# musyoku/chainer-speech-recognition

Hardware: AMD Instinct MI355X
Metric: utterances/sec (T=1000, 40x3 feat, |V|~3000) CTC train step (higher is better)
Workload: dtype bf16

## Files before the change

### chainer-speech-recognition_amd/asr/_lib.py

```python
import ctypes
import os

import torch

_HERE = os.path.dirname(os.path.abspath(__file__))
_ACT = os.environ.get("ASR_ACT", "").lower()
LIB_PATH = os.environ.get("ASR_HIP_LIB") or os.path.join(os.path.dirname(_HERE),
                                                        "libasr_hip_f16.so" if _ACT in ("f16", "fp16", "float16", "half") else "libasr_hip.so")

_lib = None


def act_dtype():
    return torch.float16 if lib().asr_act_dtype() else torch.bfloat16


def debug_flag(key, default):
    for item in os.environ.get("ASR_DEBUG", "").split(","):
        k, _, v = item.strip().partition("=")
        if k == key and v:
            return int(v)
    return default

c_void_p, c_int, c_float, c_size_t = ctypes.c_void_p, ctypes.c_int, ctypes.c_float, ctypes.c_size_t
# ... 39 lines not shown
    "asr_conv_nt_8pn_ok": (c_int, [c_void_p, c_void_p, c_int, c_void_p, c_int, c_void_p] + [c_int] * 9),
    "asr_conv_nt_8pn": (c_int, [c_void_p, c_void_p, c_void_p, c_int, c_void_p, c_int, c_void_p] + [c_int] * 12),
    "asr_conv_direct_ok": (c_int, [c_int] * 11),
    "asr_conv_direct_nt": (c_int, [c_void_p, c_void_p, c_void_p, c_int, c_void_p, c_void_p] + [c_int] * 12),
    "asr_conv_mp_ok": (c_int, [c_int] * 5),
    "asr_conv_mp_fwd": (c_int, [c_void_p] * 3 + [c_int] + [c_void_p] * 3 + [c_int] * 11),
    "asr_conv_mp_bwd_workspace": (c_longlong, [c_int] * 5),
    "asr_conv_mp_bwd": (c_int, [c_void_p] * 7 + [c_int] * 12),
    "asr_pack_input_pad": (c_int, [c_void_p, c_void_p, c_int] + [c_longlong] * 4 + [c_int] * 5 + [c_void_p]),
    "asr_conv_weight_pack_bwd": (c_int, [c_void_p] * 3 + [c_int] * 4),
    "asr_gemm_tn_acc": (c_int, [c_void_p, c_void_p, c_int, c_void_p, c_int, c_void_p, c_int] + [c_int] * 3),
    "asr_gemm_tn_acc_group": (c_int, [c_void_p, c_int] + [c_void_p] * 9),
    "asr_gemm_tn_8ph_ok": (c_int, [c_void_p, c_int, c_void_p, c_int, c_void_p, c_int, c_int, c_int, c_int]),
    "asr_gemm_tn_acc_group_8ph": (c_int, [c_void_p, c_int] + [c_void_p] * 9),
    "asr_cast_bf16": (c_int, [c_void_p, c_void_p, c_void_p, c_int, c_int, c_int]),
    "asr_cast_bf16_many": (c_int, [c_void_p, c_void_p, c_int, c_longlong]),
    "asr_bf16_to_f32": (c_int, [c_void_p, c_void_p, c_void_p, c_longlong]),
    "asr_permute4": (c_int, [c_void_p, c_void_p, c_int, c_void_p, c_int] + [c_int] * 4 + [c_longlong] * 4),
    "asr_im2col": (c_int, [c_void_p, c_void_p, c_int] + [c_longlong] * 4 + [c_int] * 10 + [c_void_p]),
    "asr_col2im": (c_int, [c_void_p, c_void_p] + [c_int] * 10 + [c_void_p]),
    "asr_activation_fwd": (c_int, [c_void_p] * 3 + [c_longlong, c_int, c_float]),
    "asr_activation_bwd": (c_int, [c_void_p] * 4 + [c_longlong, c_int, c_float]),
    "asr_glu_fwd": (c_int, [c_void_p] * 3 + [c_longlong, c_int]),
    "asr_glu_bwd": (c_int, [c_void_p] * 4 + [c_longlong, c_int]),
    "asr_dropout": (c_int, [c_void_p] * 3 + [c_longlong, c_float, ctypes.c_uint]),
    "asr_conv_weight_pack": (c_int, [c_void_p] * 3 + [c_int] * 6),
    "asr_conv_weight_grad_unpack": (c_int, [c_void_p] * 3 + [c_int] * 6),
    "asr_conv_tn_acc": (c_int, [c_void_p, c_void_p, c_int, c_void_p, c_void_p] + [c_int] * 12),
    "asr_conv_tn_8ph_ok": (c_int, [c_void_p, c_int, c_void_p, c_void_p] + [c_int] * 10),
    "asr_conv_tn_acc_8ph": (c_int, [c_void_p, c_void_p, c_int, c_void_p, c_void_p] + [c_int] * 12),
    "asr_conv_tn_copies": (c_int, [c_int] * 4),
    "asr_conv_tn_acc_copies": (c_int, [c_void_p, c_void_p, c_int, c_void_p, c_void_p] + [c_int] * 13),
    "asr_conv_weight_grad_unpack_copies": (c_int, [c_void_p, c_void_p, c_int, c_void_p] + [c_int] * 6),
    "asr_maxout2_fwd": (c_int, [c_void_p] * 3 + [c_longlong]),
    "asr_maxout2_bwd": (c_int, [c_void_p] * 4 + [c_longlong]),
    "asr_maxout2_pool_fwd": (c_int, [c_void_p] * 3 + [c_longlong, c_int, c_int, c_int]),
    "asr_maxout2_pool_bwd": (c_int, [c_void_p] * 4 + [c_longlong, c_int, c_int, c_int]),
    "asr_maxout2_pool_bwd_db": (c_int, [c_void_p] * 5 + [c_longlong, c_int, c_int, c_int]),
    "asr_maxout2_pool_bwd_db_ok": (c_int, [c_int]),
    "asr_maxpool_h_fwd": (c_int, [c_void_p] * 3 + [c_longlong, c_int, c_int, c_int]),
    "asr_maxpool_h_bwd": (c_int, [c_void_p] * 4 + [c_longlong, c_int, c_int, c_int]),
    "asr_add_bf16": (c_int, [c_void_p] * 4 + [c_longlong]),
    "asr_colsum_acc": (c_int, [c_void_p, c_void_p, c_int, c_longlong, c_int, c_int, c_void_p]),
    "asr_layernorm_fwd": (c_int, [c_void_p, c_void_p, c_int, c_void_p, c_int] + [c_void_p] * 4 + [c_longlong, c_int, c_int]),
    "asr_layernorm_fwd_lse": (c_int, [c_void_p] * 8 + [c_longlong, c_int]),
    "asr_layernorm_fwd_lse_ok": (c_int, [c_int, c_int]),
    "asr_layernorm_bwd": (c_int, [c_void_p, c_void_p, c_int, c_void_p, c_int] + [c_void_p] * 3 + [c_void_p, c_int, c_void_p, c_void_p,
                                  c_longlong, c_int, c_int]),
    "asr_layernorm_bwd_rows_ws_bytes": (c_longlong, [c_longlong, c_int]),
    "asr_layernorm_bwd_rows": (c_int, [c_void_p] * 7 + [c_int, c_void_p, c_void_p, c_longlong, c_int, c_int, c_void_p, c_longlong]),
    "asr_layernorm_fold_partials": (c_int, [c_void_p, c_void_p, c_int, c_int, c_int, c_void_p, c_void_p, c_void_p]),
    "asr_layernorm_ctc_bwd_ws_bytes": (c_longlong, [c_int, c_int, c_int]),
    "asr_layernorm_ctc_bwd": (c_int, [c_void_p] * 7 + [c_int, c_void_p, c_void_p, c_int, c_int, c_int, c_void_p, c_longlong, c_int] +
                              [c_void_p, c_int, c_int, c_void_p, c_void_p, c_int, c_float] * 2 + [c_void_p]),
    "asr_weightnorm_fwd": (c_int, [c_void_p] * 5 + [c_int, c_int]),
    "asr_weightnorm_bwd": (c_int, [c_void_p] * 7 + [c_int, c_int]),
    "asr_channel_stats": (c_int, [c_void_p, c_void_p, c_longlong, c_int, c_void_p, c_void_p]),
    "asr_channel_affine": (c_int, [c_void_p] * 5 + [c_longlong, c_int]),
    "asr_weightnorm_init": (c_int, [c_void_p] * 5 + [c_int]),
    "asr_gru_sync_bytes": (c_size_t, [c_int] * 3),
    "asr_gru_fwd_accepts_bf16_gi": (c_int, [c_int] * 5),
    "asr_gru_gates_f16_ok": (c_int, [c_int] * 5),
    "asr_gru_fwd": (c_int, [c_void_p, c_void_p, c_int] + [c_void_p] * 6 + [c_int] * 4 + [c_void_p, c_int, c_void_p, c_int]),
    "asr_gru_bwd": (c_int, [c_void_p] * 10 + [c_int] * 4 + [c_void_p, c_int, c_void_p, c_void_p, c_int]),
    "asr_gru_fwd_state": (c_int, [c_void_p] * 9 + [c_int] * 4 + [c_void_p]),
    "asr_gru_bwd_state": (c_int, [c_void_p] * 13 + [c_int] * 4 + [c_void_p, c_void_p]),
# ... 71 lines not shown
```

### chainer-speech-recognition_amd/asr/_ops.py

```python
import os

import torch

from . import _lib
from ._lib import check, ptr, stream

BF16 = _lib.act_dtype()
F32 = torch.float32


def _is_bf16(t):
    if t.dtype == BF16:
        return 1
    if t.dtype == F32:
        return 0
    raise TypeError("expected float32 or bfloat16, got %s" % t.dtype)


def gemm_nt(a, b, bias=None, out_dtype=BF16, out=None):
    assert a.dtype == BF16 and b.dtype == BF16 and a.dim() == 2 and b.dim() == 2
    assert a.stride(1) == 1 and b.stride(1) == 1 and a.shape[1] == b.shape[1]
    M, K = a.shape
    N = b.shape[0]
    if out is None:
# ... 112 lines not shown
    return dx


def conv_weight_pack(W, transpose=False, Kp=None):
    assert W.dtype == F32 and W.is_contiguous() and W.dim() == 4
    Co, Ci, KH, KW = W.shape
    Kp = (KH * KW * Ci + 7) // 8 * 8 if Kp is None else int(Kp)
    dst = torch.empty((Kp, Co) if transpose else (Co, Kp), dtype=BF16, device=W.device)
    check(_lib.lib().asr_conv_weight_pack(stream(), ptr(W), ptr(dst), Co, Ci, KH, KW, Kp, int(transpose)), "asr_conv_weight_pack")
    return dst


def conv_weight_grad_unpack(scratch, gW, channel_pitch=0):
    Co, Ci, KH, KW = gW.shape
    assert scratch.dtype == F32 and scratch.is_contiguous() and gW.is_contiguous()
    copies = scratch.shape[0] if scratch.dim() == 3 else 1
    check(_lib.lib().asr_conv_weight_grad_unpack_copies(stream(), ptr(scratch), copies, ptr(gW), Co, Ci, KH, KW, scratch.shape[-1],
                                                        int(channel_pitch)), "asr_conv_weight_grad_unpack_copies")


def conv_tn_copies(Co, Cs, KH, KW):
    return int(_lib.lib().asr_conv_tn_copies(int(Co), int(Cs), int(KH), int(KW)))


def conv_tn_acc(g2, x, scratch, KH, KW, pad_h, pad_t, Tr, Hr):
    Ts, B, Hs, Cs = x.shape
    Co = g2.shape[1]
    assert x.dtype == BF16 and g2.dtype == BF16 and scratch.dtype == F32 and g2.shape[0] == Tr * B * Hr
    copies = scratch.shape[0] if scratch.dim() == 3 else 1
    assert tuple(scratch.shape[-2:]) == (Co, KH * KW * Cs) and scratch.is_contiguous() and copies in (1, 8)
    rc = _lib.lib().asr_conv_tn_acc_copies(stream(), ptr(g2), g2.stride(0), ptr(x), ptr(scratch), scratch.shape[-1], copies, Co, Ts, B,
                                           Hs, Cs, KH, KW, pad_h, pad_t, Tr, Hr)
    check(rc, "asr_conv_tn_acc_copies")


def conv_tn_acc_8ph(g2, x, scratch, KH, KW, pad_h, pad_t, Tr, Hr):
    Ts, B, Hs, Cs = x.shape
    Co = g2.shape[1]
    assert tuple(scratch.shape) == (Co, KH * KW * Cs) and scratch.is_contiguous()
    rc = _lib.lib().asr_conv_tn_acc_8ph(stream(), ptr(g2), g2.stride(0), ptr(x), ptr(scratch), scratch.shape[-1], Co, Ts, B, Hs, Cs, KH, KW,
                                        pad_h, pad_t, Tr, Hr)
    check(rc, "asr_conv_tn_acc_8ph")


ACT_KINDS = {"relu": 0, "clipped_relu": 1, "leaky_relu": 2, "elu": 3, "sigmoid": 4, "tanh": 5, "hard_sigmoid": 6,
             "softplus": 7}


def activation_fwd(x, kind, alpha=0.0):
    assert x.dtype == BF16 and x.is_contiguous()
    y = torch.empty_like(x)
    check(_lib.lib().asr_activation_fwd(stream(), ptr(x), ptr(y), x.numel(), ACT_KINDS[kind], float(alpha)), "asr_activation_fwd")
    return y


def activation_bwd(x, dy, kind, alpha=0.0):
    dx = torch.empty_like(x)
    check(_lib.lib().asr_activation_bwd(stream(), ptr(x), ptr(dy.contiguous()), ptr(dx), x.numel(), ACT_KINDS[kind],
                                        float(alpha)), "asr_activation_bwd")
    return dx


def glu_fwd(x):
    assert x.dtype == BF16 and x.is_contiguous() and x.shape[-1] % 2 == 0
    C = x.shape[-1] // 2
    y = torch.empty(x.shape[:-1] + (C,), dtype=BF16, device=x.device)
# ... 761 lines not shown
```

### chainer-speech-recognition_amd/asr/functions.py

```python
import math
import os

import torch

from . import _ops
from ._lib import debug_flag as _lib_debug
from .link import grad_buffer, grads_queued

BF16, F32 = _ops.BF16, torch.float32


_SIDE = {"streams": {}, "origins": {}, "enabled": True, "dirty": set(), "keep": [], "keep_bytes": 0,
         "join_before_recurrence": _lib_debug("side_join", 0) != 0}
_KEEP_LIMIT = 512
_KEEP_BYTES_LIMIT = int(_lib_debug("side_keep_gb", 48)) << 30


def side_stream():
    if not _SIDE["enabled"]:
        return None
    cur = torch.cuda.current_stream()
    key = cur.cuda_stream
    st = _SIDE["streams"].get(key)
    if st is None:
# ... 273 lines not shown
                pointwise = False
        if not pointwise:
            col = _ops.im2col(x, (x.stride(3), x.stride(0), x.stride(2), x.stride(1)), T, B, Hin, Ci, KH, KW, pad_h,
                              pad_t, Tout)
        y = _ops.gemm_nt(col, w16, b.detach() if b is not None else None, F32 if out_f32 else BF16)
        ctx.save_for_backward(col, w16t, wbwd)
        ctx.params = (W, b)
        ctx.meta = (B, Ci, Hin, T, Co, KH, KW, pad_h, pad_t, Tout, Hout, pointwise, x.dtype, ctx.needs_input_grad[0], False)
        if out_f32:
            ctx._asr_mailbox = _GradMailbox(y)
        ctx._asr_biasbox = _BiasBox(y, b)
        return y.reshape(Tout, B, Hout, Co)

    @staticmethod
    def backward(ctx, gy):
        col, w16t, wbwd = ctx.saved_tensors
        W, b = ctx.params
        B, Ci, Hin, T, Co, KH, KW, pad_h, pad_t, Tout, Hout, pointwise, xdtype, need_dx, implicit = ctx.meta
        bias_done = _take_bias_done(ctx)
        gy, gy_auto = _incoming_bf16(ctx, gy, Co)
        g2 = gy.reshape(Tout * B * Hout, Co)
        Kreal = KH * KW * Ci
        xphys = col if implicit else None
        Kp = (Kreal + 7) // 8 * 8 if implicit else col.shape[1]
        w_is_param = isinstance(W, torch.nn.Parameter)
        if w_is_param:
            gW = grad_buffer(W)
        else:
            gW = torch.empty(W.shape, dtype=F32, device=gy.device)
            _ops.fill_(gW, 0.0)
        gb = grad_buffer(b) if b is not None else None

        def weight_grads():
            if implicit:
                Cs = xphys.shape[3]
                copies = _ops.conv_tn_copies(Co, Cs, KH, KW)
                scratch = torch.empty((copies, Co, KH * KW * Cs) if copies > 1 else (Co, KH * KW * Cs), dtype=F32, device=gy.device)
                _ops.fill_(scratch, 0.0)
                _ops.conv_tn_acc(g2, xphys, scratch, KH, KW, pad_h, pad_t, Tout, Hout)
                _ops.conv_weight_grad_unpack(scratch, gW, Cs)
            elif Kp == Kreal and KH == 1 and KW == 1:
                _ops.gemm_tn_acc(g2, col, gW.reshape(Co, Kreal))
            else:
                scratch = torch.empty((Co, Kp), dtype=F32, device=gy.device)
                _ops.fill_(scratch, 0.0)
                _ops.gemm_tn_acc(g2, col, scratch)
                _ops.conv_weight_grad_unpack(scratch, gW)
            if gb is not None:
                if not bias_done:
                    _ops.colsum_acc(g2, gb)
                elif gy_auto is not None and getattr(ctx, "_asr_mailbox", None) is not None:
                    _ops.colsum_acc(gy_auto, gb)

        def input_grad():
            if not need_dx:
                return None
            if (not pointwise and KH == Hin and Hout == 1 and KW == 1 and pad_h == 0 and pad_t == 0 and Tout == T
                    and w16t.shape[0] == Kreal):
                gp = _ops.gemm_nt(g2, w16t, None, BF16).reshape(T, B, Hin, Ci)
            elif wbwd is not None and not pointwise:
                gp = _ops.conv_nt(g2.reshape(Tout, B, Hout, Co), wbwd, None, BF16, KH, KW, pad_h, pad_t, -1, T, Hin).reshape(T, B, Hin, Ci)
            else:
                dcol = _ops.gemm_nt(g2, w16t, None, BF16)
                gp = dcol.reshape(T, B, Hin, Ci) if pointwise else _ops.col2im(dcol, T, B, Hin, Ci, KH, KW, pad_h, pad_t, Tout)
            if xdtype == F32:
                return _ops.bf16_to_f32(gp).permute(1, 3, 2, 0)
            return gp.permute(1, 3, 2, 0)

        if w_is_param:
            with _OnSide(g2, col, gy_auto):
                weight_grads()
            gx = input_grad()
            grads_queued(W, b)
        else:
            gx = input_grad()
            weight_grads()
            grads_queued(b)
        return gx, (None if w_is_param else gW), None, None, None, None, None, None, None, None, None


def conv_weight_matrix(W):
    return _ops.conv_weight_pack(W.contiguous())

# ... 807 lines not shown
```

### chainer-speech-recognition_amd/csrc/gemm.hip

```cpp
#include "common.hpp"
#include "../../include/asr_hip.h"

namespace asr {
namespace gemm {

typedef short bf16x8 __attribute__((ext_vector_type(8)));
typedef short bf16x4 __attribute__((ext_vector_type(4)));
typedef float f32x4 __attribute__((ext_vector_type(4)));

constexpr int BM = 128, BN = 128, BK = 64;
constexpr int NT_LDS_BYTES = 2 * (BM + BN) * BK * 2;

__device__ __forceinline__ void tile_of(int bid, int tiles_m, int tiles_n_signed, int& tm, int& tn) {
    const int tiles_n = tiles_n_signed < 0 ? -tiles_n_signed : tiles_n_signed;
    if (tiles_n_signed > 0) {
        tm = bid / tiles_n;
        tn = bid - tm * tiles_n;
        return;
    }
    const int full = (tiles_m >> 3) << 3;
    if (bid < full * tiles_n) {
        const int x = bid & 7, idx = bid >> 3;
        tm = (idx / tiles_n) * 8 + x;
        tn = idx - (idx / tiles_n) * tiles_n;
// ... 1456 lines not shown
        if (lda[i] < M[i] || ldb[i] < N[i] || ldc[i] < N[i]) return ASR_ERR_BAD_ARG;
        vec = vec && tn_vec_ok(A[i], lda[i], B[i], ldb[i], M[i], N[i], K[i]);
        TnProb& q = grp.p[i];
        q.A = (const uint16_t*)A[i]; q.B = (const uint16_t*)B[i]; q.C = C[i];
        q.lda = lda[i]; q.ldb = ldb[i]; q.ldc = ldc[i]; q.M = M[i]; q.N = N[i]; q.K = K[i];
        q.tiles_n = cdiv(N[i], BN);
        tiles += cdiv(M[i], BM) * q.tiles_n;
        q.tile_end = tiles;
        kmax = K[i] > kmax ? K[i] : kmax;
    }
    grp.n = n;
    hipStream_t stream = (hipStream_t)stream_;
    int k_per_split;
    static int target = 0;
    if (!target) { target = debug_flag("tn_group_target", 1152); if (target < 1) target = 1152; }
    const int splits = tn_splits(tiles, kmax, k_per_split, target, true);
    const TnProb& q = grp.p[0];
    if (vec)
        hipLaunchKernelGGL(gemm_tn_vec_kernel<false>, dim3(tn_grid(tiles, splits)), dim3(256), TN_LDS_BYTES, stream,
                           q.A, q.lda, q.B, q.ldb, q.C, q.ldc, q.M, q.N, q.K, q.tiles_n, k_per_split, grp, ConvDesc{}, 0LL);
    else
        hipLaunchKernelGGL(gemm_tn_kernel<false>, dim3(tn_grid(tiles, splits)), dim3(256), TN_LDS_BYTES, stream,
                           q.A, q.lda, q.B, q.ldb, q.C, q.ldc, q.M, q.N, q.K, q.tiles_n, k_per_split, ConvDesc{}, 0LL, grp);
    ASR_LAUNCH_CHECK();
    return ASR_OK;
}

extern "C" int asr_conv_tn_copies(int Co, int Cs, int KH, int KW) {
    const int N = KH * KW * Cs;
    if (tn256_ok(Co, 8, 8, nullptr, nullptr, true)) return 1;
    return cdiv(Co, BM) * cdiv(N, BN) <= 2 ? 8 : 1;
}

extern "C" int asr_conv_tn_acc_copies(void* stream_, const void* g, int ldg, const void* x, float* C, int ldc, int copies, int Co, int Ts,
                                      int B, int Hs, int Cs, int KH, int KW, int pad_h, int pad_t, int Tr, int Hr) {
    if (!g || !x || !C || Co <= 0 || Ts <= 0 || B <= 0 || Hs <= 0 || Cs <= 0 || KH <= 0 || KW <= 0 || Tr <= 0 || Hr <= 0)
        return ASR_ERR_BAD_ARG;
    const int N = KH * KW * Cs;
    const long long K = (long long)Tr * B * Hr;
    if (ldg < Co || ldc < N || (copies != 1 && copies != 8)) return ASR_ERR_BAD_ARG;
    if (copies == 8 && asr_conv_tn_copies(Co, Cs, KH, KW) != 8) return ASR_ERR_BAD_ARG;
    if ((Cs & 7) || K > 0x7fffffffLL || (((uintptr_t)x) & 15)) return ASR_ERR_UNSUPPORTED;
    hipStream_t stream = (hipStream_t)stream_;
    {
        static const int use8 = debug_flag("tn_8ph", 1), tn256_forced = debug_flag("tn256", 1);
        if (use8 && tn256_forced != 2 && copies == 1 && Co >= 192 && N >= 192 && K >= 2048 &&
            asr_conv_tn_8ph_ok(g, ldg, x, C, ldc, Co, Ts, B, Hs, Cs, KH, KW, Tr, Hr))
            return asr_conv_tn_acc_8ph(stream_, g, ldg, x, C, ldc, Co, Ts, B, Hs, Cs, KH, KW, pad_h, pad_t, Tr, Hr);
    }
    const ConvDesc cd{B, Hs, Cs, Ts, KH, KW, pad_h, pad_t, +1, Hr};
    if (tn256_ok(Co, ldg, 8, g, x, true)) {
        const int t2m = cdiv(Co, T2M), t2n = cdiv(N, T2N);
        int kps;
        const int sp = tn_splits(t2m * t2n, (int)K, kps);
        static bool attr = false;
        if (!attr) { (void)hipFuncSetAttribute((const void*)gemm_tn256_kernel<true>, hipFuncAttributeMaxDynamicSharedMemorySize, TN2_LDS_BYTES); attr = true; }
        hipLaunchKernelGGL(gemm_tn256_kernel<true>, dim3(8 * t2m * t2n * cdiv(sp, 8)), dim3(256), TN2_LDS_BYTES, stream,
                           (const uint16_t*)g, ldg, (const uint16_t*)x, 0, C, ldc, Co, N, (int)K, t2n, kps, cd);
        ASR_LAUNCH_CHECK();
        return ASR_OK;
    }
    const int tiles_m = cdiv(Co, BM), tiles_n = cdiv(N, BN);
    int k_per_split;
    const int splits = tn_splits(tiles_m * tiles_n, (int)K, k_per_split);
    const unsigned long long x_bytes = (unsigned long long)Ts * B * Hs * Cs * 2;
    if (tn_vec_ok(g, ldg, x, 8, Co, N, (int)K) && x_bytes < 0xfffffff0ull) {
        hipLaunchKernelGGL(gemm_tn_vec_kernel<true>, dim3(tn_grid(tiles_m * tiles_n, splits)), dim3(256), TN_LDS_BYTES, stream,
                           (const uint16_t*)g, ldg, (const uint16_t*)x, 0, C, ldc, Co, N, (int)K, tiles_n, k_per_split, TnGroup{}, cd,
                           copies == 8 ? (long long)Co * ldc : 0LL);
        ASR_LAUNCH_CHECK();
        return ASR_OK;
    }
    hipLaunchKernelGGL(gemm_tn_kernel<true>, dim3(tn_grid(tiles_m * tiles_n, splits)), dim3(256), TN_LDS_BYTES, stream,
                       (const uint16_t*)g, ldg, (const uint16_t*)x, 0, C, ldc, Co, N, (int)K, tiles_n, k_per_split, cd, copies == 8 ? (long long)Co * ldc : 0LL,
                       TnGroup{});
    ASR_LAUNCH_CHECK();
// ... 103 lines not shown
```

### include/asr_hip.h

```cpp
#ifndef ASR_HIP_H
#define ASR_HIP_H
#include <stddef.h>
#include <stdint.h>
#ifdef __cplusplus
extern "C" {
#endif

int asr_version(void);
int asr_act_dtype(void);
int asr_stream_delay(void* stream, int microseconds);
int asr_occupy_cus(void* stream, int microseconds, int lds_bytes, int blocks);
int asr_stream_traffic(void* stream, int microseconds, int lds_bytes, int blocks, void* buf, long long bytes);

size_t asr_ctc_workspace_bytes(int T, int B, int V, int Lmax, int gram);
int asr_ctc_forward(void* stream, const float* xs, const int32_t* label_unigram, const int32_t* label_bigram,
                    const int32_t* x_len, const int32_t* l_len, int T, int B, int V, int Lmax, int blank,
                    float* loss_per_utt, float* loss_mean, void* workspace, size_t workspace_bytes);
int asr_ctc_forward_lse(void* stream, const float* xs, const int32_t* label_unigram, const int32_t* label_bigram,
                        const int32_t* x_len, const int32_t* l_len, int T, int B, int V, int Lmax, int blank, float* loss_per_utt,
                        float* loss_mean, void* workspace, size_t workspace_bytes, const float* row_lse);
int asr_ctc_backward(void* stream, const float* xs, const int32_t* x_len, int T, int B, int V, int Lmax, int gram,
                     const float* gy, int gy_per_utt, float scale, float* grad, const void* workspace,
                     size_t workspace_bytes);
int asr_ctc_loss_grad(void* stream, const float* xs, const int32_t* label_unigram, const int32_t* label_bigram,
// ... 55 lines not shown
                int Hs, int Cs, int KH, int KW, int pad_h, int pad_t, int sgn, int Tr, int Hr, int N);
int asr_conv_nt_8ph_ok(const void* x, const void* W, int ldw, const void* out, int out_bf16, const float* bias, int Ts, int B, int Hs, int Cs,
                       int KH, int KW, int Tr, int Hr, int N);
int asr_conv_nt_8ph(void* stream, const void* x, const void* W, int ldw, void* out, int out_bf16, const float* bias, int Ts, int B, int Hs,
                    int Cs, int KH, int KW, int pad_h, int pad_t, int sgn, int Tr, int Hr, int N);
int asr_conv_nt_8pn_ok(const void* x, const void* W, int ldw, const void* out, int out_bf16, const float* bias, int Ts, int B, int Hs, int Cs,
                       int KH, int KW, int Tr, int Hr, int N);
int asr_conv_nt_8pn(void* stream, const void* x, const void* W, int ldw, void* out, int out_bf16, const float* bias, int Ts, int B, int Hs,
                    int Cs, int KH, int KW, int pad_h, int pad_t, int sgn, int Tr, int Hr, int N);
int asr_conv_direct_ok(int Ts, int B, int Hs, int Cs, int KH, int KW, int Tr, int Hr, int N, int K, int out_bf16);
int asr_conv_direct_nt(void* stream, const void* x, const void* W, int ldw, void* out, const float* bias, int Ts, int B, int Hs, int Cs,
                       int KH, int KW, int pad_h, int pad_t, int sgn, int Tr, int Hr, int N);
int asr_conv_mp_ok(int Ci, int KH, int KW, int Co, int k);
int asr_conv_mp_fwd(void* stream, const void* x8, const void* W, int ldw, const float* bias, void* y, void* idx, int Ts, int B, int Hs,
                    int KH, int KW, int pad_h, int pad_t, int Tout, int Hout, int Co, int k);
long long asr_conv_mp_bwd_workspace(int Tout, int B, int Hout, int Co, int k);
int asr_conv_mp_bwd(void* stream, const void* gy, const void* idx, const void* x8, void* workspace, float* gW, float* gb, int Ts, int B,
                    int Hs, int Ci, int KH, int KW, int pad_h, int pad_t, int Tout, int Hout, int Co, int k);
int asr_pack_input_pad(void* stream, const void* x, int x_bf16, long long sT, long long sB, long long sH, long long sC, int T,
                       int B, int H, int C, int Cpad, void* out_bf16);
int asr_conv_weight_pack_bwd(void* stream, const float* W, void* dst, int Co, int Ci, int KH, int KW);
int asr_conv_tn_acc(void* stream, const void* g, int ldg, const void* x, float* C, int ldc, int Co, int Ts, int B, int Hs,
                    int Cs, int KH, int KW, int pad_h, int pad_t, int Tr, int Hr);
int asr_conv_tn_8ph_ok(const void* g, int ldg, const void* x, const float* C, int ldc, int Co, int Ts, int B, int Hs, int Cs, int KH, int KW,
                       int Tr, int Hr);
int asr_conv_tn_acc_8ph(void* stream, const void* g, int ldg, const void* x, float* C, int ldc, int Co, int Ts, int B, int Hs, int Cs, int KH,
                        int KW, int pad_h, int pad_t, int Tr, int Hr);
int asr_conv_weight_grad_unpack(void* stream, const float* scratch, float* gW, int Co, int Ci, int KH, int KW, int Kp, int Cs);
int asr_conv_tn_copies(int Co, int Cs, int KH, int KW);
int asr_conv_tn_acc_copies(void* stream, const void* g, int ldg, const void* x, float* C, int ldc, int copies, int Co, int Ts, int B,
                           int Hs, int Cs, int KH, int KW, int pad_h, int pad_t, int Tr, int Hr);
int asr_conv_weight_grad_unpack_copies(void* stream, const float* scratch, int copies, float* gW, int Co, int Ci, int KH, int KW, int Kp,
                                       int Cs);
int asr_maxout2_fwd(void* stream, const void* x, void* y, long long n_out);
int asr_maxout2_bwd(void* stream, const void* x, const void* dy, void* dx, long long n_out);
int asr_maxout2_pool_fwd(void* stream, const void* x, void* y, long long R, int Hin, int C, int k);
int asr_maxout2_pool_bwd(void* stream, const void* x, const void* dy, void* dx, long long R, int Hin, int C, int k);
int asr_maxout2_pool_bwd_db(void* stream, const void* x, const void* dy, void* dx, float* db, long long R, int Hin, int C, int k);
int asr_maxout2_pool_bwd_db_ok(int C);
int asr_maxpool_h_fwd(void* stream, const void* x, void* y, long long R, int Hin, int C, int k);
int asr_maxpool_h_bwd(void* stream, const void* x, const void* dy, void* dx, long long R, int Hin, int C, int k);
int asr_add_bf16(void* stream, const void* a, const void* b, void* y, long long n);
int asr_activation_fwd(void* stream, const void* x, void* y, long long n, int kind, float alpha);
int asr_activation_bwd(void* stream, const void* x, const void* dy, void* dx, long long n, int kind, float alpha);
int asr_glu_fwd(void* stream, const void* x, void* y, long long rows, int C);
int asr_glu_bwd(void* stream, const void* x, const void* dy, void* dx, long long rows, int C);
int asr_dropout(void* stream, const void* x, void* y, long long n, float ratio, unsigned int seed);
int asr_colsum_acc(void* stream, const void* x, int x_bf16, long long rows, int cols, int ld, float* out);

int asr_layernorm_fwd(void* stream, const void* x, int x_bf16, void* y, int y_bf16, const float* gamma,
                      const float* beta, float* mean, float* rstd, long long rows, int D, int C);
int asr_layernorm_fwd_lse(void* stream, const float* x, float* y, const float* gamma, const float* beta, float* mean, float* rstd,
                          float* lse, long long rows, int D);
int asr_layernorm_fwd_lse_ok(int D, int C);
int asr_layernorm_bwd(void* stream, const void* x, int x_bf16, const void* dy, int dy_bf16, const float* gamma,
                      const float* mean, const float* rstd, void* dx, int dx_bf16, float* dgamma, float* dbeta,
                      long long rows, int D, int C);
long long asr_layernorm_bwd_rows_ws_bytes(long long rows, int D);
int asr_layernorm_bwd_rows(void* stream, const float* x, const float* dy, const float* gamma, const float* mean,
                           const float* rstd, void* dx, int dx_bf16, float* dgamma, float* dbeta, long long rows, int D,
                           int C, void* ws, long long ws_bytes);

int asr_weightnorm_fwd(void* stream, const float* V, const float* g, float* W, float* norm, int Co, int K);
int asr_weightnorm_bwd(void* stream, const float* gW, const float* V, const float* g, const float* norm, float* gV,
                       float* gg, int Co, int K);
int asr_channel_stats(void* stream, const float* x, long long rows, int C, float* mean, float* stdv);
// ... 85 lines not shown
```

Baseline: 2465.

## Add direct implicit conv weight-gradient kernel with fused bias column-sum

Adds a dedicated HIP MFMA kernel that computes conv weight gradients directly from the physical input layout. Several kernel-width taps are handled per block with shared A tiles, XCD-aware walkers and atomic accumulation. When a bias gradient is pending, it is folded into the same kernel via an MFMA against a ones vector, skipping the separate colsum pass. The kernel is routed by default for small Co or small K shapes. The risks are atomic contention and double-buffered tiles that use a lot of LDS.

```diff
diff --git a/chainer-speech-recognition_amd/asr/_lib.py b/chainer-speech-recognition_amd/asr/_lib.py
--- a/chainer-speech-recognition_amd/asr/_lib.py
+++ b/chainer-speech-recognition_amd/asr/_lib.py
@@ -95,6 +95,9 @@
     "asr_conv_tn_copies": (c_int, [c_int] * 4),
     "asr_conv_tn_acc_copies": (c_int, [c_void_p, c_void_p, c_int, c_void_p, c_void_p] + [c_int] * 13),
     "asr_conv_weight_grad_unpack_copies": (c_int, [c_void_p, c_void_p, c_int, c_void_p] + [c_int] * 6),
+    "asr_conv_wgrad_direct_ok": (c_int, [c_int] * 9),
+    "asr_conv_wgrad_direct_routed": (c_int, [c_int] * 9),
+    "asr_conv_wgrad_direct": (c_int, [c_void_p, c_void_p, c_int, c_void_p, c_void_p, c_int, c_int, c_void_p] + [c_int] * 11),
     "asr_maxout2_fwd": (c_int, [c_void_p] * 3 + [c_longlong]),
     "asr_maxout2_bwd": (c_int, [c_void_p] * 4 + [c_longlong]),
     "asr_maxout2_pool_fwd": (c_int, [c_void_p] * 3 + [c_longlong, c_int, c_int, c_int]),
diff --git a/chainer-speech-recognition_amd/asr/_ops.py b/chainer-speech-recognition_amd/asr/_ops.py
--- a/chainer-speech-recognition_amd/asr/_ops.py
+++ b/chainer-speech-recognition_amd/asr/_ops.py
@@ -168,6 +168,30 @@
     rc = _lib.lib().asr_conv_tn_acc_copies(stream(), ptr(g2), g2.stride(0), ptr(x), ptr(scratch), scratch.shape[-1], copies, Co, Ts, B,
                                            Hs, Cs, KH, KW, pad_h, pad_t, Tr, Hr)
     check(rc, "asr_conv_tn_acc_copies")
+
+
+def conv_wgrad_direct_ok(Co, x, KH, KW, Tr, Hr):
+    Ts, B, Hs, Cs = x.shape
+    return bool(_lib.lib().asr_conv_wgrad_direct_ok(int(Co), Ts, B, Hs, Cs, KH, KW, Tr, Hr))
+
+
+def conv_wgrad_direct_routed(Co, x, KH, KW, Tr, Hr):
+    Ts, B, Hs, Cs = x.shape
+    return bool(_lib.lib().asr_conv_wgrad_direct_routed(int(Co), Ts, B, Hs, Cs, KH, KW, Tr, Hr))
+
+
+def conv_wgrad_direct(g2, x, scratch, db, KH, KW, pad_h, pad_t, Tr, Hr):
+    Ts, B, Hs, Cs = x.shape
+    Co = g2.shape[1]
+    assert x.dtype == BF16 and g2.dtype == BF16 and scratch.dtype == F32 and g2.shape[0] == Tr * B * Hr and x.is_contiguous()
+    copies = scratch.shape[0] if scratch.dim() == 3 else 1
+    assert tuple(scratch.shape[-2:])[0] == Co and scratch.shape[-1] >= KH * KW * Cs and scratch.stride(-1) == 1 and copies in (1, 8)
+    assert db is None or (db.dtype == F32 and db.numel() == Co and db.is_contiguous())
+    rc = _lib.lib().asr_conv_wgrad_direct(stream(), ptr(g2), g2.stride(0), ptr(x), scratch.data_ptr(), scratch.stride(-2), copies,
+                                          ptr(db) if db is not None else None, Co, Ts, B, Hs, Cs, KH, KW, pad_h, pad_t, Tr, Hr)
+    if rc != -3:
+        check(rc, "asr_conv_wgrad_direct")
+    return rc
 
 
 def conv_tn_acc_8ph(g2, x, scratch, KH, KW, pad_h, pad_t, Tr, Hr):
diff --git a/chainer-speech-recognition_amd/asr/functions.py b/chainer-speech-recognition_amd/asr/functions.py
--- a/chainer-speech-recognition_amd/asr/functions.py
+++ b/chainer-speech-recognition_amd/asr/functions.py
@@ -329,12 +329,18 @@
         gb = grad_buffer(b) if b is not None else None
 
         def weight_grads():
+            bias_in_product = False
             if implicit:
                 Cs = xphys.shape[3]
                 copies = _ops.conv_tn_copies(Co, Cs, KH, KW)
                 scratch = torch.empty((copies, Co, KH * KW * Cs) if copies > 1 else (Co, KH * KW * Cs), dtype=F32, device=gy.device)
                 _ops.fill_(scratch, 0.0)
-                _ops.conv_tn_acc(g2, xphys, scratch, KH, KW, pad_h, pad_t, Tout, Hout)
+                if (gb is not None and not bias_done and g2.stride(0) % 8 == 0
+                        and _ops.conv_wgrad_direct_routed(Co, xphys, KH, KW, Tout, Hout)
+                        and _ops.conv_wgrad_direct(g2, xphys, scratch, gb.reshape(-1), KH, KW, pad_h, pad_t, Tout, Hout) == 0):
+                    bias_in_product = True
+                else:
+                    _ops.conv_tn_acc(g2, xphys, scratch, KH, KW, pad_h, pad_t, Tout, Hout)
                 _ops.conv_weight_grad_unpack(scratch, gW, Cs)
             elif Kp == Kreal and KH == 1 and KW == 1:
                 _ops.gemm_tn_acc(g2, col, gW.reshape(Co, Kreal))
@@ -345,7 +351,8 @@
                 _ops.conv_weight_grad_unpack(scratch, gW)
             if gb is not None:
                 if not bias_done:
-                    _ops.colsum_acc(g2, gb)
+                    if not bias_in_product:
+                        _ops.colsum_acc(g2, gb)
                 elif gy_auto is not None and getattr(ctx, "_asr_mailbox", None) is not None:
                     _ops.colsum_acc(gy_auto, gb)
 
diff --git a/chainer-speech-recognition_amd/csrc/conv_wgrad.hip b/chainer-speech-recognition_amd/csrc/conv_wgrad.hip
--- /dev/null
+++ b/chainer-speech-recognition_amd/csrc/conv_wgrad.hip
@@ -0,0 +1,323 @@
+#include <hip/hip_runtime.h>
+#include <stdint.h>
+
+#include <type_traits>
+
+#include "common.hpp"
+
+namespace asr {
+namespace convw {
+
+typedef short bf16x8 __attribute__((ext_vector_type(8)));
+typedef short bf16x4 __attribute__((ext_vector_type(4)));
+typedef float f32x4 __attribute__((ext_vector_type(4)));
+typedef unsigned int u32x4 __attribute__((ext_vector_type(4)));
+union Frag {
+    bf16x8 v;
+    bf16x4 h[2];
+};
+
+__device__ __forceinline__ bf16x4 lds_tr16(const char* p) {
+    return __builtin_amdgcn_ds_read_tr16_b64_v4i16((__attribute__((address_space(3))) bf16x4*)p);
+}
+
+struct Desc {
+    int B, Hs, Cs, Ts, KH, KW, ph, pt, Hr, Tr, Co, ldg, ldc;
+    int Tt, ntiles;
+    int kwg, nco, nci;
+    int groups, walkers;
+    int xr;
+    int xbuf;
+    long long copy_stride;
+};
+
+constexpr int ROWS = 128;
+constexpr int NX = 3;
+constexpr unsigned OOB = 0xfffffff0u;
+
+template <int MT, int WN, int NTAP>
+__global__ __launch_bounds__(512, 1) void conv_wgrad_kernel(const uint16_t* __restrict__ g, const uint16_t* __restrict__ x, float* __restrict__ C,
+                                                            float* __restrict__ db, Desc d, unsigned g_bytes, unsigned x_bytes) {
+    extern __shared__ __attribute__((aligned(16))) char smem[];
+    constexpr int WM = 8 / WN, COC = MT * 16 * WM, CIC = WN * 16, PBA = COC * 2, PBX = CIC * 2;
+    constexpr int NPA = COC / 16, NPX = CIC / 16;
+    constexpr int CHA = COC / 8, CHX = CIC / 8;
+    constexpr int NA = ROWS * CHA / 512;
+    constexpr int ABYTES = ROWS * PBA;
+    auto swz = [](int row, int np) { return np >= 8 ? (row & 7) : np == 4 ? ((row >> 1) & 3) : np == 2 ? ((row >> 2) & 1) : 0; };
+    const int tid = threadIdx.x, lane = tid & 63, wid = __builtin_amdgcn_readfirstlane(tid >> 6);
+    const int wm = wid / WN, wn = wid % WN;
+    const int bufbytes = ABYTES + d.xbuf;
+
+    const int xcd = blockIdx.x & 7;
+    int j = blockIdx.x >> 3;
+    const int piece = j % d.groups;
+    const int walker = (j / d.groups) * 8 + xcd;
+    int pc = piece;
+    const int ci_chunk = pc % d.nci; pc /= d.nci;
+    const int co_chunk = pc % d.nco; pc /= d.nco;
+    const int kwgi = pc % d.kwg;
+    const int kh = pc / d.kwg;
+    const int kw0 = kwgi * NTAP;
+    const int cobase = co_chunk * COC, cibase = ci_chunk * CIC;
+    C += (size_t)xcd * d.copy_stride;
+
+    const __amdgpu_buffer_rsrc_t rsrc_g = __builtin_amdgcn_make_buffer_rsrc((void*)g, 0, (int)g_bytes, 0x00020000);
+    const __amdgpu_buffer_rsrc_t rsrc_x = __builtin_amdgcn_make_buffer_rsrc((void*)x, 0, (int)x_bytes, 0x00020000);
+
+    constexpr int RSA = 512 / CHA, RSX = 512 / CHX;
+    int a_rel[NA];
+    const int a_row0 = tid / CHA, a_c = tid % CHA;
+    const int a_lds0 = a_row0 * PBA + (((a_c >> 1) ^ swz(a_row0, NPA)) << 5) + ((a_c & 1) << 4);
+#pragma unroll
+    for (int i = 0; i < NA; ++i) {
+        const int row = a_row0 + i * RSA;
+        const int tl = row / d.Hr, h = row - tl * d.Hr;
+        a_rel[i] = ((tl * d.B * d.Hr + h) * d.ldg + cobase + a_c * 8) * 2;
+    }
+    int x_tb[NX], x_rel[NX];
+    const int x_row0 = tid / CHX, x_c = tid % CHX;
+    const int x_lds0 = ABYTES + x_row0 * PBX + (((x_c >> 1) ^ swz(x_row0, NPX)) << 5) + ((x_c & 1) << 4);
+#pragma unroll
+    for (int i = 0; i < NX; ++i) {
+        const int row = x_row0 + i * RSX;
+        const int tb = row / d.Hr, h = row - tb * d.Hr, hs = h + kh - d.ph;
+        const bool in = row < d.xr && (unsigned)hs < (unsigned)d.Hs;
+        x_tb[i] = in ? tb : (1 << 28);
+        x_rel[i] = ((tb * d.B * d.Hs + hs) * d.Cs + cibase + x_c * 8) * 2;
+    }
+    const int my_tiles = walker < d.ntiles ? (d.ntiles - walker + d.walkers - 1) / d.walkers : 0;
+    auto ask = [&](u32x4 (&ra)[NA], u32x4 (&rx)[NX], int n) {
+        const bool valid = n < my_tiles;
+        const int tile = walker + n * d.walkers;
+        const int tt = tile / d.B, b = tile - tt * d.B;
+        const int t0 = tt * d.Tt;
+        const int Mt = valid ? min(d.Tt, d.Tr - t0) * d.Hr : 0;
+        const int gbase = (t0 * d.B + b) * d.Hr * d.ldg * 2;
+        const int tx0 = t0 - d.pt + kw0;
+        const int xbase = (tx0 * d.B + b) * d.Hs * d.Cs * 2;
+#pragma unroll
+        for (int i = 0; i < NA; ++i)
+            ra[i] = __builtin_amdgcn_raw_buffer_load_b128(rsrc_g, a_row0 + i * RSA < Mt ? (unsigned)(a_rel[i] + gbase) : OOB, 0, 0);
+#pragma unroll
+        for (int i = 0; i < NX; ++i) {
+            const bool ok = valid && (unsigned)(x_tb[i] + tx0) < (unsigned)d.Ts;
+            rx[i] = __builtin_amdgcn_raw_buffer_load_b128(rsrc_x, ok ? (unsigned)(x_rel[i] + xbase) : OOB, 0, 0);
+        }
+    };
+    auto to_lds = [&](const u32x4 (&ra)[NA], const u32x4 (&rx)[NX], int buf) {
+        char* base = smem + buf * bufbytes;
+#pragma unroll
+        for (int i = 0; i < NA; ++i) *reinterpret_cast<u32x4*>(base + a_lds0 + i * RSA * PBA) = ra[i];
+#pragma unroll
+        for (int i = 0; i < NX; ++i)
+            if (x_row0 + i * RSX < d.xr) *reinterpret_cast<u32x4*>(base + x_lds0 + i * RSX * PBX) = rx[i];
+    };
+
+    const int gq = lane >> 4, q = (lane >> 2) & 3, p = lane & 3;
+    int offa[MT][2], offx[NTAP][2];
+#pragma unroll
+    for (int hf = 0; hf < 2; ++hf) {
+        const int row = 16 * hf + 4 * gq + q;
+#pragma unroll
+        for (int i = 0; i < MT; ++i) offa[i][hf] = row * PBA + (((wm * MT + i) ^ swz(row, NPA)) << 5) + p * 8;
+#pragma unroll
+        for (int t = 0; t < NTAP; ++t) {
+            const int rx = row + t * d.Hr;
+            offx[t][hf] = ABYTES + rx * PBX + ((wn ^ swz(rx, NPX)) << 5) + p * 8;
+        }
+    }
+    int offb[2];
+#pragma unroll
+    for (int hf = 0; hf < 2; ++hf) {
+        const int row = 16 * hf + 4 * gq + q;
+        offb[hf] = row * PBA + (((wm * MT + (wn < MT ? wn : 0)) ^ swz(row, NPA)) << 5) + p * 8;
+    }
+    f32x4 acc[MT][NTAP], accb = {0.f, 0.f, 0.f, 0.f};
+#pragma unroll
+    for (int i = 0; i < MT; ++i)
+#pragma unroll
+        for (int t = 0; t < NTAP; ++t) acc[i][t] = (f32x4){0.f, 0.f, 0.f, 0.f};
+    const bool do_bias = db != nullptr && kh == 0 && kwgi == 0 && ci_chunk == 0 && wn < MT;
+    Frag ones;
+#pragma unroll
+    for (int e = 0; e < 8; ++e) ones.v[e] = (short)(ASR_ACT_IS_F16 ? 0x3c00 : 0x3f80);
+
+    auto work = [&](int buf) {
+        const char* base = smem + buf * bufbytes;
+        Frag a[MT], bx[NTAP];
+#pragma unroll
+        for (int i = 0; i < MT; ++i) {
+            a[i].h[0] = lds_tr16(base + offa[i][0]);
+            a[i].h[1] = lds_tr16(base + offa[i][1]);
+        }
+#pragma unroll
+        for (int t = 0; t < NTAP; ++t) {
+            bx[t].h[0] = lds_tr16(base + offx[t][0]);
+            bx[t].h[1] = lds_tr16(base + offx[t][1]);
+        }
+#pragma unroll
+        for (int ks = 0; ks < ROWS / 32; ++ks) {
+            constexpr int T0 = NTAP > 2 ? 2 : NTAP - 1;
+            const bool more = ks + 1 < ROWS / 32;
+#pragma unroll
+            for (int t = 0; t < T0; ++t) {
+#pragma unroll
+                for (int i = 0; i < MT; ++i) acc[i][t] = ASR_MFMA_16x16x32(a[i].v, bx[t].v, acc[i][t]);
+                if (more) {
+                    __builtin_amdgcn_sched_barrier(0);
+                    bx[t].h[0] = lds_tr16(base + offx[t][0] + (ks + 1) * 32 * PBX);
+                    bx[t].h[1] = lds_tr16(base + offx[t][1] + (ks + 1) * 32 * PBX);
+                    __builtin_amdgcn_sched_barrier(0);
+                }
+            }
+#pragma unroll
+            for (int i = 0; i < MT; ++i) {
+#pragma unroll
+                for (int t = T0; t < NTAP; ++t) acc[i][t] = ASR_MFMA_16x16x32(a[i].v, bx[t].v, acc[i][t]);
+                if (more) {
+                    __builtin_amdgcn_sched_barrier(0);
+                    a[i].h[0] = lds_tr16(base + offa[i][0] + (ks + 1) * 32 * PBA);
+                    a[i].h[1] = lds_tr16(base + offa[i][1] + (ks + 1) * 32 * PBA);
+                    __builtin_amdgcn_sched_barrier(0);
+                }
+            }
+            if (more) {
+#pragma unroll
+                for (int t = T0; t < NTAP; ++t) {
+                    bx[t].h[0] = lds_tr16(base + offx[t][0] + (ks + 1) * 32 * PBX);
+                    bx[t].h[1] = lds_tr16(base + offx[t][1] + (ks + 1) * 32 * PBX);
+                }
+                __builtin_amdgcn_sched_barrier(0);
+            }
+        }
+        if (do_bias) {
+#pragma unroll
+            for (int ks = 0; ks < ROWS / 32; ++ks) {
+                Frag s;
+                s.h[0] = lds_tr16(base + offb[0] + ks * 32 * PBA);
+                s.h[1] = lds_tr16(base + offb[1] + ks * 32 * PBA);
+                accb = ASR_MFMA_16x16x32(s.v, ones.v, accb);
+            }
+        }
+    };
+
+    u32x4 ra0[NA], rx0[NX], ra1[NA], rx1[NX];
+    ask(ra0, rx0, 0);
+    ask(ra1, rx1, 1);
+    to_lds(ra0, rx0, 0);
+    ask(ra0, rx0, 2);
+    __syncthreads();
+    for (int n = 0; n < my_tiles; n += 2) {
+        to_lds(ra1, rx1, 1);
+        ask(ra1, rx1, n + 3);
+        work(0);
+        __syncthreads();
+        to_lds(ra0, rx0, 0);
+        ask(ra0, rx0, n + 4);
+        if (n + 1 < my_tiles) work(1);
+        __syncthreads();
+    }
+
+    if (my_tiles > 0) {
+        const int r = lane & 15;
+#pragma unroll
+        for (int t = 0; t < NTAP; ++t) {
+            if (kw0 + t >= d.KW) continue;
+            const int col = (kh * d.KW + kw0 + t) * d.Cs + cibase + 16 * wn + r;
+#pragma unroll
+            for (int i = 0; i < MT; ++i)
+#pragma unroll
+                for (int reg = 0; reg < 4; ++reg) {
+                    const int co = cobase + 16 * (wm * MT + i) + 4 * gq + reg;
+                    atomicAdd(C + (size_t)co * d.ldc + col, acc[i][t][reg]);
+                }
+        }
+        if (do_bias && r == 0) {
+#pragma unroll
+            for (int reg = 0; reg < 4; ++reg) atomicAdd(db + cobase + 16 * (wm * MT + wn) + 4 * gq + reg, accb[reg]);
+        }
+    }
+}
+
+struct Plan {
+    int mt, wn, ntap;
+    Desc d;
+    size_t lds;
+    int grid;
+};
+
+static bool plan(int Co, int Ts, int B, int Hs, int Cs, int KH, int KW, int Tr, int Hr, Plan& pl) {
+    if (Co <= 0 || Co > 256 || (Co % 64) || (Cs != 32 && Cs != 64 && Cs != 128)) return false;
+    if (KH < 1 || KW < 1 || KH > 8 || KW > 8 || Hr < 1 || Hr > ROWS || Tr < 1 || Ts < 1 || B < 1 || Hs < 1) return false;
+    if ((unsigned long long)Ts * B * Hs * Cs * 2 >= 0x7ffffff0ull || (unsigned long long)Tr * B * Hr >= (1ull << 31)) return false;
+    const int wn = Cs == 32 ? 2 : 4, cic = wn * 16, wm = 8 / wn;
+    const int coc = Co % 128 == 0 ? 128 : 64;
+    const int ntap = KW <= 3 ? 3 : KW == 4 ? 4 : KW == 5 ? 5 : KW == 6 ? 3 : 4;
+    Desc& d = pl.d;
+    d.Tt = ROWS / Hr;
+    d.ntiles = B * cdiv(Tr, d.Tt);
+    d.kwg = cdiv(KW, ntap);
+    d.nco = Co / coc;
+    d.nci = Cs / cic;
+    d.groups = KH * d.kwg * d.nco * d.nci;
+    d.xr = ROWS + (ntap - 1) * Hr;
+    if (d.xr * (cic / 8) > NX * 512) return false;
+    d.xbuf = (d.xr * cic * 2 + 1023) & ~1023;
+    pl.lds = 2 * ((size_t)ROWS * coc * 2 + d.xbuf);
+    if (pl.lds > 160 * 1024) return false;
+    const int per_xcd = d.groups >= 32 ? 1 : 32 / d.groups;
+    d.walkers = 8 * per_xcd;
+    if (d.walkers > d.ntiles) d.walkers = 8 * cdiv(d.ntiles, 8);
+    pl.grid = d.groups * d.walkers;
+    pl.mt = coc / 16 / wm;
+    pl.wn = wn;
+    pl.ntap = ntap;
+    return true;
+}
+
+}
+}
+
+using namespace asr;
+using namespace asr::convw;
+
+extern "C" int asr_conv_wgrad_direct_ok(int Co, int Ts, int B, int Hs, int Cs, int KH, int KW, int Tr, int Hr) {
+    Plan pl;
+    return plan(Co, Ts, B, Hs, Cs, KH, KW, Tr, Hr, pl) ? 1 : 0;
+}
+
+extern "C" int asr_conv_wgrad_direct(void* stream_, const void* g, int ldg, const void* x, float* C, int ldc, int copies, float* db, int Co,
+                                     int Ts, int B, int Hs, int Cs, int KH, int KW, int pad_h, int pad_t, int Tr, int Hr) {
+    if (!g || !x || !C || Co <= 0 || Ts <= 0 || B <= 0 || Hs <= 0 || Cs <= 0 || KH <= 0 || KW <= 0 || Tr <= 0 || Hr <= 0) return ASR_ERR_BAD_ARG;
+    if (ldg < Co || ldc < KH * KW * Cs || (copies != 1 && copies != 8)) return ASR_ERR_BAD_ARG;
+    Plan pl;
+    if (!plan(Co, Ts, B, Hs, Cs, KH, KW, Tr, Hr, pl)) return ASR_ERR_UNSUPPORTED;
+    const unsigned long long g_bytes = ((unsigned long long)Tr * B * Hr - 1) * ldg * 2 + (unsigned long long)Co * 2;
+    if ((ldg & 7) || ((((uintptr_t)g) | ((uintptr_t)x)) & 15) || (((uintptr_t)C) & 3) || g_bytes >= 0x7ffffff0ull) return ASR_ERR_UNSUPPORTED;
+    Desc& d = pl.d;
+    d.B = B; d.Hs = Hs; d.Cs = Cs; d.Ts = Ts; d.KH = KH; d.KW = KW; d.ph = pad_h; d.pt = pad_t; d.Hr = Hr; d.Tr = Tr; d.Co = Co; d.ldg = ldg; d.ldc = ldc;
+    d.copy_stride = copies == 8 ? (long long)Co * ldc : 0LL;
+    const unsigned x_bytes = (unsigned)((unsigned long long)Ts * B * Hs * Cs * 2);
+    hipStream_t stream = (hipStream_t)stream_;
+#define ASR_CW(MT_, WN_, NT_)                                                                                                        \
+    do {                                                                                                                             \
+        static bool attr_ = false;                                                                                                   \
+        if (!attr_) {                                                                                                                \
+            (void)hipFuncSetAttribute((const void*)conv_wgrad_kernel<MT_, WN_, NT_>, hipFuncAttributeMaxDynamicSharedMemorySize, 160 * 1024); \
+            attr_ = true;                                                                                                            \
+        }                                                                                                                            \
+        hipLaunchKernelGGL((conv_wgrad_kernel<MT_, WN_, NT_>), dim3((unsigned)pl.grid), dim3(512), pl.lds, stream, (const uint16_t*)g, \
+                           (const uint16_t*)x, C, db, d, (unsigned)g_bytes, x_bytes);                                                \
+    } while (0)
+#define ASR_CWT(MT_, WN_)                                                                                                            \
+    do {                                                                                                                             \
+        if (pl.ntap == 3) ASR_CW(MT_, WN_, 3); else if (pl.ntap == 4) ASR_CW(MT_, WN_, 4); else ASR_CW(MT_, WN_, 5);                  \
+    } while (0)
+    if (pl.wn == 4) { if (pl.mt == 4) ASR_CWT(4, 4); else ASR_CWT(2, 4); }
+    else            { if (pl.mt == 2) ASR_CWT(2, 2); else ASR_CWT(1, 2); }
+#undef ASR_CWT
+#undef ASR_CW
+    ASR_LAUNCH_CHECK();
+    return ASR_OK;
+}
diff --git a/chainer-speech-recognition_amd/csrc/gemm.hip b/chainer-speech-recognition_amd/csrc/gemm.hip
--- a/chainer-speech-recognition_amd/csrc/gemm.hip
+++ b/chainer-speech-recognition_amd/csrc/gemm.hip
@@ -1512,6 +1512,15 @@
     return cdiv(Co, BM) * cdiv(N, BN) <= 2 ? 8 : 1;
 }
 
+extern "C" int asr_conv_wgrad_direct_ok(int Co, int Ts, int B, int Hs, int Cs, int KH, int KW, int Tr, int Hr);
+extern "C" int asr_conv_wgrad_direct(void* stream, const void* g, int ldg, const void* x, float* C, int ldc, int copies, float* db, int Co, int Ts,
+                                     int B, int Hs, int Cs, int KH, int KW, int pad_h, int pad_t, int Tr, int Hr);
+extern "C" int asr_conv_wgrad_direct_routed(int Co, int Ts, int B, int Hs, int Cs, int KH, int KW, int Tr, int Hr) {
+    static const int direct = debug_flag("conv_wgrad_direct", 1);
+    if (!direct || !asr_conv_wgrad_direct_ok(Co, Ts, B, Hs, Cs, KH, KW, Tr, Hr)) return 0;
+    return direct == 2 || Co < 192 || KH * KW * Cs < 192;
+}
+
 extern "C" int asr_conv_tn_acc_copies(void* stream_, const void* g, int ldg, const void* x, float* C, int ldc, int copies, int Co, int Ts,
                                       int B, int Hs, int Cs, int KH, int KW, int pad_h, int pad_t, int Tr, int Hr) {
     if (!g || !x || !C || Co <= 0 || Ts <= 0 || B <= 0 || Hs <= 0 || Cs <= 0 || KH <= 0 || KW <= 0 || Tr <= 0 || Hr <= 0)
@@ -1522,6 +1531,10 @@
     if (copies == 8 && asr_conv_tn_copies(Co, Cs, KH, KW) != 8) return ASR_ERR_BAD_ARG;
     if ((Cs & 7) || K > 0x7fffffffLL || (((uintptr_t)x) & 15)) return ASR_ERR_UNSUPPORTED;
     hipStream_t stream = (hipStream_t)stream_;
+    if (asr_conv_wgrad_direct_routed(Co, Ts, B, Hs, Cs, KH, KW, Tr, Hr)) {
+        const int rc = asr_conv_wgrad_direct(stream_, g, ldg, x, C, ldc, copies, nullptr, Co, Ts, B, Hs, Cs, KH, KW, pad_h, pad_t, Tr, Hr);
+        if (rc != ASR_ERR_UNSUPPORTED) return rc;
+    }
     {
         static const int use8 = debug_flag("tn_8ph", 1), tn256_forced = debug_flag("tn256", 1);
         if (use8 && tn256_forced != 2 && copies == 1 && Co >= 192 && N >= 192 && K >= 2048 &&
diff --git a/include/asr_hip.h b/include/asr_hip.h
--- a/include/asr_hip.h
+++ b/include/asr_hip.h
@@ -111,6 +111,10 @@
                            int Hs, int Cs, int KH, int KW, int pad_h, int pad_t, int Tr, int Hr);
 int asr_conv_weight_grad_unpack_copies(void* stream, const float* scratch, int copies, float* gW, int Co, int Ci, int KH, int KW, int Kp,
                                        int Cs);
+int asr_conv_wgrad_direct_ok(int Co, int Ts, int B, int Hs, int Cs, int KH, int KW, int Tr, int Hr);
+int asr_conv_wgrad_direct_routed(int Co, int Ts, int B, int Hs, int Cs, int KH, int KW, int Tr, int Hr);
+int asr_conv_wgrad_direct(void* stream, const void* g, int ldg, const void* x, float* C, int ldc, int copies, float* db, int Co, int Ts,
+                          int B, int Hs, int Cs, int KH, int KW, int pad_h, int pad_t, int Tr, int Hr);
 int asr_maxout2_fwd(void* stream, const void* x, void* y, long long n_out);
 int asr_maxout2_bwd(void* stream, const void* x, const void* dy, void* dx, long long n_out);
 int asr_maxout2_pool_fwd(void* stream, const void* x, void* y, long long R, int Hin, int C, int k);
```

Result: no change. 2473 (median of 6 runs) (+0.3%).
